# alvin-zyl/LDDL

Hardware: AMD Instinct MI355X
Metric: WordPiece tokens/sec (node) BERT seq128/512 at 1-8 GPUs; % HBM roofline (higher is better)
Workload: dtype u8

## Files before the change

lddl_amd/csrc/capi_tokenize.hip:

```cpp
#include "capi_ctx.h"

static int tok_debug_report(const TokParams& P, int64_t nt, hipStream_t st) {
  uint64_t h[24];
  HIP_TRY(hipMemcpyAsync(h, P.dbg, sizeof h, hipMemcpyDeviceToHost, st));
  HIP_TRY(hipStreamSynchronize(st));
  const char* nm[12] = {"loop", "setup", "classify", "except", "units", "urec", "prep", "probe", "records",
                        "tile_end", "entries", "tiles"};
  fprintf(stderr, "[lddl tok5 dbg] ntiles=%lld", (long long)nt);
  for (int k = 0; k < 12; ++k) fprintf(stderr, " %s=%llu", nm[k], (unsigned long long)h[k]);
  const char* wn[6] = {"wp_A", "wp_B", "wp_C", "wp_D", "wp_steps", "wp_lane_steps"};
  for (int k = 0; k < 6; ++k) fprintf(stderr, " %s=%llu", wn[k], (unsigned long long)h[12 + k]);
  fprintf(stderr, " prep_decode=%llu prep_dirty=%llu x_list=%llu x_load=%llu x_apply=%llu", (unsigned long long)h[18],
          (unsigned long long)h[19], (unsigned long long)h[20], (unsigned long long)h[21], (unsigned long long)h[22]);
  fprintf(stderr, "\n");
  return 0;
}

extern "C" int lddl_tokenize(lddl_ctx* c, const uint8_t* d_bytes, int64_t nbytes, const int64_t* d_sent_off,
                             int64_t n_sent, int32_t max_tok, uint16_t* d_out_ids, int64_t out_cap,
                             int32_t* d_out_ntok, int64_t* d_out_tok_off, void* stream) {
  if (!c) return set_err(LDDL_EINVAL, "null ctx");
  if (n_sent < 0 || max_tok < 1 || max_tok > 65534 || nbytes < 0 || out_cap < 0)
    return set_err(LDDL_EINVAL, "n_sent %lld nbytes %lld max_tok %d out_cap %lld", (long long)n_sent,
                   (long long)nbytes, max_tok, (long long)out_cap);
  if (!d_out_tok_off) return set_err(LDDL_EINVAL, "null device pointer");
  HIP_TRY(hipSetDevice(c->device));
  hipStream_t st = (hipStream_t)stream;
  if (n_sent == 0) {
    HIP_TRY(hipMemsetAsync(d_out_tok_off, 0, sizeof(int64_t), st));
    return 0;
  }
  if (!d_bytes || !d_sent_off || (!d_out_ids && out_cap > 0) || !d_out_ntok)
    return set_err(LDDL_EINVAL, "null device pointer");
  TokParams P{};
  P.bytes = d_bytes;
  P.sent_off = d_sent_off;
  P.n_sent = n_sent;
  P.max_tok = max_tok;
  P.out_ids = d_out_ids;
  P.out_ntok = d_out_ntok;
  P.out_tok_off = d_out_tok_off;
  P.out_cap = out_cap;
  c->spec_ids = nullptr;
  if (c->spec_flags) {
    int rc;
    if ((rc = ws_get(c, CW_SENT_SPEC, n_sent, &P.sent_spec))) return rc;
    c->spec_ids = d_out_ids;
    c->spec_ntok = d_out_ntok;
    c->spec_soff = d_sent_off;
    c->spec_nsent = n_sent;
  }
  P.top = c->d_top;
  P.pages = c->d_pages;
  P.bmp = c->d_bmp;
  P.xmap = c->d_xmap;
  P.multi = c->d_multi;
  P.slots = c->d_slots;
  P.slot_mask = c->slot_mask;
  P.bloom = c->d_bloom;
  P.pool = c->d_pool;
  P.voff = c->d_voff;
  P.maxb[0] = c->maxb[0];
  P.maxb[1] = c->maxb[1];
  for (int k = 0; k < 5; ++k) P.special[k] = c->special[k];
  P.unk = c->special[1];
  P.vt = c->d_vt;
  P.vt_mask = c->vt_mask;
  P.vbloom = c->d_vbloom;
  P.ovf = c->d_ovf;
  P.work_counter = c->d_counter;
  HIP_TRY(hipMemsetAsync(c->d_counter, 0, 64, st));
  const char* dbgenv = getenv("LDDL_TOK_DEBUG");

  if (dbgenv && dbgenv[0] == '1') {
    if (!c->d_tdbg) HIP_TRY(hipMalloc((void**)&c->d_tdbg, 32 * 8));
    HIP_TRY(hipMemsetAsync(c->d_tdbg, 0, 32 * 8, st));
    P.dbg = c->d_tdbg;
  }
  const int64_t nt = tile_count(nbytes);
  const char* eseg = getenv("LDDL_SPLIT_SEG");
  const char* ech = getenv("LDDL_SPLIT_CHUNKS");
  const int64_t seg_max = c->tok_algo == 0 ? nt : eseg && atoll(eseg) > 0 ? atoll(eseg) : SPLIT_SEG_TILES;
  const int64_t seg = nt < seg_max ? nt : seg_max;
  const bool split = c->tok_algo == 5;
  int64_t n_chunks = !split ? 1 : split_seg_slots(seg, c->n_cu) / SPLIT_CHUNK;
  if (ech && atoll(ech) > 0 && split) n_chunks = atoll(ech);
  const int64_t slots = n_chunks * SPLIT_CHUNK;
  int64_t* tile_sent;
  SplitParams S{};
  int rc;
  const int64_t fb_cap = fb_list_cap(seg, n_sent);
  if ((rc = ws_get(c, CW_TILE_SENT, nt + 1, &tile_sent)) || (rc = ws_get(c, CW_FB_LIST, (size_t)(2 * fb_cap), &S.fb_list)) ||
      (rc = ws_get(c, CW_FB_COUNT, 16, &S.fb_count)) ||
      (rc = ws_get(c, CW_ENT, (size_t)seg * 1024 + (size_t)max_tok + 4096, &S.ent)) ||
      (rc = ws_get(c, CW_SHARED_BSUM, (size_t)n_chunks + 16, &S.chunk_fill)) ||
      (rc = ws_get(c, CW_SCAN_BSUM, (size_t)scan_blocks(n_sent) + 1, &S.scan_bsum)))
// ... 27 lines not shown
```

lddl_amd/csrc/pack.hip:

```cpp
#include <algorithm>

#include "common.h"
#include "pack.h"
#include "pack_row.h"
#include "wave.h"

namespace lddl {

__global__ __launch_bounds__(1024) void scan_parts_kernel(const int64_t* a, const int64_t* b, int64_t n,
                                                          int64_t* sa, int64_t* sb, const int32_t* err,
                                                          int32_t* err_any) {
  __shared__ int64_t la[1024], lb[1024];
  __shared__ int32_t le;
  const int t = threadIdx.x;
  const int64_t per = (n + 1023) / 1024;
  const int64_t lo = min(n, t * per), hi = min(n, lo + per);
  int64_t x = 0, y = 0;
  int32_t e = 0;
  for (int64_t i = lo; i < hi; ++i) { x += a[i]; y += b[i]; e |= err[i]; }
  la[t] = x; lb[t] = y;
  if (t == 0) le = 0;
  __syncthreads();
  if (e) atomicOr(&le, e);
  for (int off = 1; off < 1024; off <<= 1) {
    int64_t u = t >= off ? la[t - off] : 0, w = t >= off ? lb[t - off] : 0;
    __syncthreads();
    la[t] += u; lb[t] += w;
    __syncthreads();
  }
  int64_t ra = la[t] - x, rb = lb[t] - y;
  for (int64_t i = lo; i < hi; ++i) { sa[i] = ra; sb[i] = rb; ra += a[i]; rb += b[i]; }
  if (t == 1023) { sa[n] = la[1023]; sb[n] = lb[1023]; *err_any = le; }
}

__global__ __launch_bounds__(256) void materialize_kernel(MatParams M) {
  __shared__ RowDesc st[4][64];
  __shared__ int64_t st_off[4][64];
  const PackView& V = M.V;
  const int lane = threadIdx.x & 63, wv = threadIdx.x >> 6;
  const int64_t total = V.pair_base[V.n_part];
  const int64_t nw = (int64_t)gridDim.x * 4;
  for (int64_t p = (int64_t)blockIdx.x * 4 + wv; p < V.n_part; p += nw) {
    const int64_t g0 = V.pair_base[p], np = V.pair_base[p + 1] - g0;
    for (int64_t c = 0; c < np; c += 64) {
      if (c + lane < np) {
        const int64_t g = g0 + c + lane;
        PairRec r;
        const RowRef w = pair_of_row(V, p, g, r);
        const int64_t off = row_tok_off(V, p, w);
        const RowDesc x = row_desc(V, r);
        st[wv][lane] = x;
        st_off[wv][lane] = off;
        store_row_meta(M, g, p, r.flags, x, total, [&] { return off; });
      }
      wave_sync();
      const int nr = (int)min((int64_t)64, np - c);
      const int hl = lane & 31;
      for (int r0 = 0; r0 < nr; r0 += 2) {
        const int rr = r0 + (lane >> 5);
        if (rr >= nr) continue;
        const RowDesc x = st[wv][rr];
        uint16_t* out = M.out_tokens + st_off[wv][rr];
        for (int t0 = 0; t0 < x.nt; t0 += 512) {
          uint16_t v[16];
#pragma unroll
          for (int k = 0; k < 16; ++k) {
            const int t = t0 + hl + 32 * k;
            uint16_t y = (uint16_t)M.sep_id;
            if (t == 0) y = (uint16_t)M.cls_id;
            else if (t <= x.l0) y = M.dense[x.src0 + (t - 1)];
            else if (t >= x.b1 && t < x.b1 + x.l1) y = M.dense[x.src1 + (t - x.b1)];
            v[k] = y;
          }
#pragma unroll
          for (int k = 0; k < 16; ++k) {
            const int t = t0 + hl + 32 * k;
            if (t < x.nt) out[t] = v[k];
          }
        }
      }
      wave_sync();
    }
  }
}

constexpr int MAT_U = 2;
constexpr int MAT_SLOW = 512;
// ... 176 lines not shown
}

hipError_t launch_chunk_parts(const int64_t* pair_base, const int64_t* doc_sent_off, const int64_t* part_doc_off,
                              int32_t dup, int64_t n_part, int32_t* chunk_part, int64_t* part_pb, hipStream_t s) {
  const int64_t nblk = std::max<int64_t>(1, std::min<int64_t>((n_part + 255) / 256, 1024));
  hipLaunchKernelGGL(chunk_parts_kernel, dim3((unsigned)nblk), dim3(256), 0, s, pair_base, doc_sent_off, part_doc_off,
                     dup, n_part, chunk_part, part_pb);
  return hipGetLastError();
}

constexpr int RS_U = 2;
__global__ __launch_bounds__(256) void rowspan_kernel(MatParams M, int64_t total) {
  const PackView& V = M.V;
  const int lane = threadIdx.x & 63, wv = threadIdx.x >> 6;
  const int64_t gbase = ((int64_t)blockIdx.x * 4 + wv) * 64 * RS_U;
  if (gbase >= total) return;
  int64_t g[RS_U], p[RS_U], at[RS_U];
  bool in[RS_U];
#pragma unroll
  for (int u = 0; u < RS_U; ++u) {
    g[u] = gbase + 64 * u + lane;
    in[u] = g[u] < total;
    p[u] = in[u] ? M.chunk_part[(gbase >> 6) + u] : 0;
  }
#pragma unroll
  for (int u = 0; u < RS_U; ++u) {
    if (in[u]) p[u] = part_walk(V, p[u], g[u]);
    at[u] = in[u] ? M.part_pb[p[u]] + (g[u] - V.pair_base[p[u]]) : 0;
  }
  SpanRec t[RS_U];
  int64_t off[RS_U];
#pragma unroll
  for (int u = 0; u < RS_U; ++u) t[u] = M.span[at[u]];
  if (M.out_tok_off) {
#pragma unroll
    for (int u = 0; u < RS_U; ++u) off[u] = V.tok_base[p[u]] + V.tok_local[at[u]];
  }
#pragma unroll
  for (int u = 0; u < RS_U; ++u) {
    if (!in[u]) continue;
    M.out_src0[g[u]] = t[u].src0;
    M.out_src1[g[u]] = t[u].src1;
    store_row_meta(M, g[u], p[u], t[u].flags, row_desc(t[u]), total, [&] { return off[u]; });
  }
}

hipError_t launch_row_spans(const MatParams& M, int64_t total_pairs, hipStream_t s) {
  const int64_t nblk = (total_pairs + 256 * RS_U - 1) / (256 * RS_U);
  hipLaunchKernelGGL(rowspan_kernel, dim3((unsigned)nblk), dim3(256), 0, s, M, total_pairs);
  return hipGetLastError();
}

constexpr int SCAN_ITEMS = 4096;

__host__ __device__ int64_t scan_blocks(int64_t n) { return (n + SCAN_ITEMS - 1) / SCAN_ITEMS; }

__device__ __forceinline__ int64_t block_excl_scan256(int64_t v, int64_t* red, int64_t* total) {
  const int lane = threadIdx.x & 63, w = threadIdx.x >> 6;
  int64_t x = v;
#pragma unroll
  for (int o = 1; o < 64; o <<= 1) {
    const int64_t y = __shfl_up(x, o);
    if (lane >= o) x += y;
  }
  if (lane == 63) red[w] = x;
  __syncthreads();
  int64_t pre = 0, tot = 0;
#pragma unroll
  for (int k = 0; k < 4; ++k) {
    if (k < w) pre += red[k];
    tot += red[k];
  }
  __syncthreads();
  *total = tot;
  return pre + x - v;
}

__device__ __forceinline__ void scan_range(const int64_t* d_lo, const int64_t* d_hi, int64_t n, int64_t& lo,
                                           int64_t& hi) {
  lo = d_lo ? *d_lo : 0;
  hi = d_lo ? *d_hi : n;
}

__global__ __launch_bounds__(256) void scan_reduce_kernel(const int32_t* ntok, const int64_t* d_lo, const int64_t* d_hi,
                                                          int64_t n, int64_t* bsum) {
  __shared__ int64_t red[4];
  int64_t lo, hi;
  scan_range(d_lo, d_hi, n, lo, hi);
  const int64_t b0 = lo + (int64_t)blockIdx.x * SCAN_ITEMS;
  if (b0 >= hi) return;
  int64_t sum = 0;
  for (int k = threadIdx.x; k < SCAN_ITEMS; k += 256)
    if (b0 + k < hi) sum += ntok[b0 + k];
  int64_t tot;
  block_excl_scan256(sum, red, &tot);
  if (threadIdx.x == 0) bsum[blockIdx.x] = tot;
}

__global__ __launch_bounds__(256) void scan_bsum_kernel(int64_t* bsum, const int64_t* d_lo, const int64_t* d_hi,
                                                        int64_t n, const int64_t* tokoff) {
  __shared__ int64_t red[4];
  int64_t lo, hi;
  scan_range(d_lo, d_hi, n, lo, hi);
  const int64_t nb = scan_blocks(hi - lo);
  int64_t carry = d_lo ? tokoff[lo] : 0;
  for (int64_t c = 0; c < nb; c += 256) {
    const int64_t i = c + threadIdx.x;
    const int64_t v = i < nb ? bsum[i] : 0;
    int64_t tot;
    const int64_t ex = block_excl_scan256(v, red, &tot);
    if (i < nb) bsum[i] = carry + ex;
    carry += tot;
  }
  if (threadIdx.x == 0) bsum[nb] = carry;
}

__global__ __launch_bounds__(256) void scan_write_kernel(const int32_t* ntok, const int64_t* d_lo, const int64_t* d_hi,
                                                         int64_t n, const int64_t* bsum, int64_t* tokoff) {
  __shared__ int64_t red[4];
  int64_t lo, hi;
  scan_range(d_lo, d_hi, n, lo, hi);
  if (lo + (int64_t)blockIdx.x * SCAN_ITEMS >= hi) return;
  const int64_t b0 = lo + (int64_t)blockIdx.x * SCAN_ITEMS + threadIdx.x * 16;
  int32_t v[16];
  int64_t sum = 0;
#pragma unroll
  for (int k = 0; k < 16; ++k) {
    v[k] = b0 + k < hi ? ntok[b0 + k] : 0;
    sum += v[k];
  }
  int64_t tot;
  int64_t run = bsum[blockIdx.x] + block_excl_scan256(sum, red, &tot);
  __shared__ int64_t ob[SCAN_ITEMS + SCAN_ITEMS / 16];
#pragma unroll
  for (int k = 0; k < 16; ++k) {
    ob[threadIdx.x * 17 + k] = run;
    run += v[k];
  }
  __syncthreads();
  const int64_t c0 = lo + (int64_t)blockIdx.x * SCAN_ITEMS;
#pragma unroll
  for (int k = 0; k < 16; ++k) {
    const int j = k * 256 + threadIdx.x;
    if (c0 + j < hi) tokoff[c0 + j] = ob[j + (j >> 4)];
  }
  if (lo + ((int64_t)blockIdx.x + 1) * SCAN_ITEMS >= hi && threadIdx.x == 0) tokoff[hi] = bsum[scan_blocks(hi - lo)];
}

static hipError_t scan_launch(const int32_t* ntok, const int64_t* d_lo, const int64_t* d_hi, int64_t n,
                              int64_t* tokoff, int64_t* blocksums, hipStream_t s) {
  const int64_t nb = scan_blocks(n);
  if (nb == 0) return d_lo ? hipSuccess : hipMemsetAsync(tokoff, 0, sizeof(int64_t), s);
  hipLaunchKernelGGL(scan_reduce_kernel, dim3((unsigned)nb), dim3(256), 0, s, ntok, d_lo, d_hi, n, blocksums);
  hipLaunchKernelGGL(scan_bsum_kernel, dim3(1), dim3(256), 0, s, blocksums, d_lo, d_hi, n, (const int64_t*)tokoff);
  hipLaunchKernelGGL(scan_write_kernel, dim3((unsigned)nb), dim3(256), 0, s, ntok, d_lo, d_hi, n,
                     (const int64_t*)blocksums, tokoff);
  return hipGetLastError();
}

hipError_t launch_scan_ntok(const int32_t* ntok, int64_t n, int64_t* tokoff, int64_t* blocksums, hipStream_t s) {
  return scan_launch(ntok, nullptr, nullptr, n, tokoff, blocksums, s);
}

hipError_t launch_scan_ntok_range(const int32_t* ntok, const int64_t* d_lo, const int64_t* d_hi, int64_t max_items,
                                  int64_t* tokoff, int64_t* blocksums, hipStream_t s) {
  return scan_launch(ntok, d_lo, d_hi, max_items, tokoff, blocksums, s);
}

hipError_t launch_scan_parts(const int64_t* a, const int64_t* b, int64_t n, int64_t* sa, int64_t* sb,
                             const int32_t* err, int32_t* err_any, hipStream_t s) {
  hipLaunchKernelGGL(scan_parts_kernel, dim3(1), dim3(1024), 0, s, a, b, n, sa, sb, err, err_any);
  return hipGetLastError();
}

__global__ __launch_bounds__(256) void sent_special_kernel(const uint16_t* ids, const int64_t* tok_off,
                                                           const int32_t* ntok, int64_t n_sent, uint32_t cls,
                                                           uint32_t sep, uint8_t* out) {
  for (int64_t s = (int64_t)blockIdx.x * blockDim.x + threadIdx.x; s < n_sent; s += (int64_t)gridDim.x * blockDim.x) {
    const uint16_t* t = ids + tok_off[s];
    const int n = ntok[s];
    uint32_t f = 0;
    for (int k = 0; k < n; ++k) {
      const uint32_t v = t[k];
      f |= (v == cls) | (v == sep);
    }
    out[s] = (uint8_t)f;
  }
}

__global__ __launch_bounds__(256) void masked_lm_kernel(MlmParams M) {
  const int sl = threadIdx.x & 15;
  const int64_t total = M.V.pair_base[M.V.n_part];
  const int64_t ng = (int64_t)gridDim.x * 16;
  for (int64_t g = (int64_t)blockIdx.x * 16 + (threadIdx.x >> 4); g < total; g += ng) {
    const int64_t p = M.row_part[g];
    const MaskRef m = mask_ref(M, p, row_ref(M.V, p, g));
    uint16_t* row = M.tokens + M.tok_off[g];
    if (sl == 0) store_mask_off(M, g, total, m);
    for (int k = sl; k < m.nm; k += 16) {
      const uint32_t e = M.marena[m.aoff + k];
      const uint32_t pos = e & 0xFFFFu, nid = e >> 16;
      const uint16_t label = row[pos];
      M.out_pos[m.ooff + k] = (uint16_t)pos;
      M.out_label[m.ooff + k] = label;
      if (nid != MLM_KEEP) row[pos] = (uint16_t)nid;
    }
  }
}

constexpr int MLM_SPAN_UNROLL = 8;

__global__ __launch_bounds__(256) void masked_lm_spans_kernel(MlmParams M) {
  struct RowLds {
    int64_t aoff[64], ooff[64], a[64], b[64];
    int32_t l0[64], pre[65];
  };
  __shared__ RowLds R[4];
  const int lane = threadIdx.x & 63, wv = threadIdx.x >> 6;
  RowLds& L = R[wv];
  const int64_t total = M.V.pair_base[M.V.n_part];
  const int64_t nw = (int64_t)gridDim.x * 4;
  for (int64_t g0 = ((int64_t)blockIdx.x * 4 + wv) * 64; g0 < total; g0 += nw * 64) {
    const int64_t g = g0 + lane;
    int nm = 0;
    if (g < total) {
      const int64_t p = M.row_part[g];
      const MaskRef m = mask_ref(M, p, row_ref(M.V, p, g));
      nm = m.nm;
      L.aoff[lane] = m.aoff;
      L.ooff[lane] = m.ooff;
      L.a[lane] = M.src0[g];
      L.b[lane] = M.src1[g];
      L.l0[lane] = M.len0[g];
      store_mask_off(M, g, total, m);
    }
    const int incl = wave_incl_add(nm);
    L.pre[lane] = incl - nm;
    if (lane == 63) L.pre[64] = incl;
    const int T = lane_get(incl, 63);
    wave_sync();
    int r = 0;
    constexpr int U = MLM_SPAN_UNROLL;
    for (int t0 = 0; t0 < T; t0 += 64 * U) {
      int rr[U], kk[U];
      uint32_t e[U];
#pragma unroll
      for (int u = 0; u < U; ++u) {
        const int t = t0 + 64 * u + lane;
        rr[u] = -1;
// ... 64 lines not shown
```

lddl_amd/csrc/tokenize.h:

```cpp
#pragma once
#include <hip/hip_runtime.h>
#include <stdint.h>

namespace lddl {

constexpr int WB_OVF = 384;
constexpr int TOK_WAVES = 4;
constexpr int BLOOM_WORDS = 8192;

struct TokParams {
  const uint8_t* bytes;
  const int64_t* sent_off;
  int64_t n_sent;
  int32_t max_tok;
  uint16_t* out_ids;
  int32_t* out_ntok;
  int64_t* out_tok_off;
  int64_t out_cap;
  uint8_t* sent_spec;
  const uint16_t* top;
  const uint32_t* pages;
  const uint4* multi;
  const uint32_t* bmp;
  const uint32_t* xmap;
  const uint4* slots;
  const uint32_t* bloom;
  uint32_t slot_mask;
  const uint8_t* pool;
  const uint32_t* voff;
  uint32_t maxb[2];
  uint32_t special[5];
  uint32_t unk;
  const uint4* vt;
  uint32_t vt_mask;
  const uint32_t* vbloom;
  uint8_t* ovf;
  uint32_t* work_counter;
  uint64_t* dbg;
};

int64_t tile_count(int64_t nbytes);
hipError_t launch_tile_bounds(const int64_t* sent_off, int64_t n_sent, int64_t n_tiles, int64_t* tile_sent,
                              hipStream_t s, int64_t seg = 0, int sup = 1);
hipError_t launch_tokenize_fallback(const TokParams& P, const int64_t* fb_list, const int32_t* fb_count,
                                    int64_t fb_cap, int grid, hipStream_t s);
const void* tokenize_fallback_kernel_ptr();
hipError_t launch_list_all_tiles(int64_t n_tiles, const int64_t* tile_sent, int64_t* fb_list, int32_t* fb_count,
                                 int64_t fb_cap, hipStream_t s);
inline int64_t fb_list_cap(int64_t seg_tiles, int64_t n_sent) {
  return 2 * seg_tiles + 64 + (n_sent + 30) / 31;
}

constexpr int64_t SPLIT_SEG_TILES = int64_t(1) << 23;
constexpr uint32_t SPLIT_CHUNK = 1024;
constexpr uint32_t SPLIT_EDEF = 0xF000u;
constexpr uint16_t SPLIT_NENT_FB = 0xFFFFu;
constexpr uint16_t SPLIT_EHOLE = 0xFFFFu;

struct SplitParams {
  int64_t seg_tiles;
  int64_t t0, t1;
  const int64_t* tile_sent;
  uint16_t* ent;
  uint4* rec;
  uint4* pcs;
  uint4* pch;
  uint32_t* chunk_fill;
  uint32_t* chunk_ctr;
  uint32_t n_chunks;
  uint2* smeta;
  uint16_t* snslot;
  uint8_t* cnt8;
  int64_t* scan_bsum;
  int64_t seg_sent_cap;
  int64_t* fb_list;
  int32_t* fb_count;
  int64_t fb_cap;
  uint32_t* n_fallback;
  unsigned long long* n_rec;
};
struct SplitTiming {
  hipEvent_t ev[3][2][64];
  int n[3];
};
hipError_t launch_tokenize_split(const TokParams& P, int64_t nbytes, int64_t* tile_sent, SplitParams S, int n_cu,
                                 int fb_grid, hipStream_t s, SplitTiming* tm = nullptr);
hipError_t launch_tokenize_serial_dense(const TokParams& P, int64_t nbytes, int64_t* tile_sent, SplitParams S,
                                        int n_cu, int fb_grid, hipStream_t s);
int64_t split_seg_slots(int64_t seg_tiles, int n_cu);

}
```

lddl_amd/csrc/tokenize_split.hip:

```cpp
#include <string.h>

#include "common.h"
#include "tokenize.h"
#include "wave.h"
#include "tokenize_serial.h"
#include "pack.h"


namespace lddl {
namespace tok5 {

constexpr int CAP = 2048;
constexpr int DCAP = 256;
constexpr int SCAN_OCC = 5;
#ifndef LDDL_SCAN_SUPER
#define LDDL_SCAN_SUPER 16
#endif
constexpr int SUPER = LDDL_SCAN_SUPER;
#ifndef LDDL_SCAN_FK
#define LDDL_SCAN_FK 2
#endif
constexpr int FK = LDDL_SCAN_FK;
#ifndef LDDL_SCAN_FKEY
#define LDDL_SCAN_FKEY 16
// ... 1219 lines not shown
        put_piece(0, (uint32_t)P.unk);
        np = 1;
        finish();
      } else {
        const int len = e - s;
        const int lc = min(len, 24);
        auto msk = [&](int k, uint32_t cc) {
          const int nbk = min(max(lc - 4 * k, 0), 4);
          return cc & (nbk >= 4 ? 0xFFFFFFFFu : ((1u << (8 * nbk)) - 1u));
        };
        const uint32_t m0c = msk(0, c0), m1c = msk(1, c1), m2c = msk(2, c2), m3c = msk(3, c3), m4c = msk(4, c4),
                       m5c = msk(5, c5);
        const uint32_t want = ((uint32_t)len << 16) | (cont << 24) | 0x80000000u;
        bool m0 = (((a1.z & 0xFFFF0000u) ^ want) | (a0.x ^ m0c) | (a0.y ^ m1c) | (a0.z ^ m2c) | (a0.w ^ m3c) |
                   (a1.x ^ m4c) | (a1.y ^ m5c)) == 0u;
        bool m1 = (((b1.z & 0xFFFF0000u) ^ want) | (b0.x ^ m0c) | (b0.y ^ m1c) | (b0.z ^ m2c) | (b0.w ^ m3c) |
                   (b1.x ^ m4c) | (b1.y ^ m5c)) == 0u;
        if (len > 24) {
          if (m0)
            for (int k = 24; k < len; ++k) m0 = m0 && kbyte(s + k) == P.pool[a1.w + k];
          if (m1)
            for (int k = 24; k < len; ++k) m1 = m1 && kbyte(s + k) == P.pool[b1.w + k];
        }
        if (m0 || m1) {
          put_piece(np, (m0 ? a1.z : b1.z) & 0xFFFFu);
          ++np;
          s = e;
          if (s >= we) {
            finish();
          } else {
            cont = 1;
            start_piece(mb1);
          }
        } else if (!(a1.z & 0x80000000u) || !(b1.z & 0x80000000u)) {
          bslot = -1;
          shrink();
        } else {
          bslot = (int)(((uint32_t)bslot + 1u) & vmask);
        }
      }
    }
    WP_STAMP(2)
    if (pr >= 0) {
      if (q0.x == 0u) {
        pr = -1;
      } else if ((q0.x & 0xFFu) > 24u && !qlong) {
        q2 = *recq(S, 2, (uint32_t)pr);
        q3 = *recq(S, 3, (uint32_t)pr);
        qlong = true;
      } else if (r < 0) {
        const int len = (int)(q0.x & 0xFFu);
        kb[0] = q0.z; kb[64] = q0.w;
        kb[128] = q1.x; kb[192] = q1.y; kb[256] = q1.z; kb[320] = q1.w;
        kb[384] = q2.x; kb[448] = q2.y; kb[512] = q2.z; kb[576] = q2.w;
        kb[640] = q3.x; kb[704] = q3.y; kb[768] = q3.z; kb[832] = q3.w;
        kb[896] = 0u;
        kb[960] = 0u;
        r = pr;
        pr = -1;
        ++nrec;
        s = 0;
        we = len;
        np = 0;
        cont = 0;
        start_piece(mb0);
      }
    }
    WP_STAMP(3)
    if (wdbg) {
      wacc[4] += 1;
      wacc[5] += __popcll(__ballot(r >= 0));
    }
    if (__ballot(r >= 0 || pr >= 0) == 0 && u >= nun) break;
  }
  if (wdbg && lane == 0)
    for (int k = 0; k < 6; ++k) atomicAdd((unsigned long long*)&P.dbg[12 + k], (unsigned long long)wacc[k]);
#undef WP_STAMP
  if (S.n_rec) {
    const uint32_t tot = lane_get(wave_incl_add(nrec), 63);
    if (lane == 0 && tot) atomicAdd(S.n_rec, (unsigned long long)tot);
  }
}

constexpr int CNT_U = 4;
__global__ __launch_bounds__(256) void count_kernel(TokParams P, SplitParams S) {
  const int64_t sA = S.tile_sent[S.t0], sB = S.tile_sent[S.t1];
  const int64_t stride = (int64_t)gridDim.x * 256 * CNT_U;
  for (int64_t s0 = sA + (int64_t)blockIdx.x * 256 * CNT_U + threadIdx.x; s0 < sB; s0 += stride) {
    uint2 m[CNT_U];
    int32_t t[CNT_U];
    uint32_t n[CNT_U];
#pragma unroll
    for (int u = 0; u < CNT_U; ++u) {
      const int64_t s = s0 + 256 * u;
      const bool in = s < sB;
      m[u] = in ? S.smeta[s] : make_uint2(SPLIT_NENT_FB, 0u);
      t[u] = in ? P.out_ntok[s] : 0;
      n[u] = in ? S.snslot[s] : 0u;
    }
#pragma unroll
    for (int u = 0; u < CNT_U; ++u) {
      if ((m[u].x & 0xFFFFu) != SPLIT_NENT_FB) {
        const uint32_t q = m[u].y + (m[u].x >> 16);
        for (uint32_t k = 0; k < n[u]; ++k) t[u] += S.cnt8[q + k];
        t[u] = min(t[u], P.max_tok);
      }
    }
#pragma unroll
    for (int u = 0; u < CNT_U; ++u)
      if (s0 + 256 * u < sB) P.out_ntok[s0 + 256 * u] = t[u];
  }
}

struct ExpSent {
  int64_t eb;
  int64_t dst;
  uint32_t qb;
  uint32_t lim;
  uint32_t e0;
  uint32_t pad;
};
struct ExpLds {
  ExpSent sn[64];
  uint32_t hf[64];
};

template <bool ALL_DIRECT>
__global__ __launch_bounds__(256) void expand_kernel(TokParams P, SplitParams S) {
  __shared__ ExpLds X[4];
  const int lane = threadIdx.x & 63;
  const int wv = __builtin_amdgcn_readfirstlane(threadIdx.x >> 6);
  ExpLds& E = X[wv];
  const int64_t sA = uni64(S.tile_sent[S.t0]), sB = uni64(S.tile_sent[S.t1]);
  const int64_t base = P.sent_off[0], ebase = S.t0 << 10;
  const int64_t nwaves = (int64_t)gridDim.x * 4;
  typedef uint32_t u32x3 __attribute__((ext_vector_type(3)));
  const uint4* const pcs = S.pcs;
  const uint4* const pch = S.pch;
  uint32_t tag = 0;
  E.hf[lane] = 0u;
  for (int64_t g0 = sA + ((int64_t)blockIdx.x * 4 + wv) * 64; g0 < sB; g0 += nwaves * 64) {
    const int64_t s = g0 + lane;
    uint32_t ne = 0;
    int64_t eoff = 0, d = 0;
    uint32_t qb = 0, lim = 0;
    if (s < sB) {
      const uint2 m = S.smeta[s];
      const int32_t nt = P.out_ntok[s];
      ne = m.x & 0xFFFFu;
      if (ne == SPLIT_NENT_FB) ne = (uint32_t)nt;
      d = P.out_tok_off[s];
      eoff = P.sent_off[s] - base - ebase;
      qb = (m.x & 0xFFFFu) == SPLIT_NENT_FB ? 0u : m.y;
      lim = (uint32_t)max((int64_t)0, min((int64_t)nt, P.out_cap - d));
    }
    const uint32_t x = wave_incl_add(ne);
    const uint32_t e0 = x - ne;
    const uint32_t T = lane_get(x, 63);
    ExpSent es;
    es.eb = eoff - (int64_t)e0;
    es.dst = d;
    es.qb = qb;
    es.lim = lim;
    es.e0 = e0;
    es.pad = 0;
    const uint64_t nzm = __ballot(ne != 0);
    if (ne != 0) E.sn[bits_below(nzm)] = es;
    uint32_t hcar = 0;
    auto owner = [&](uint32_t st) -> uint32_t {
      ++tag;
      if (ne != 0 && e0 - st < 64u) E.hf[e0 - st] = tag;
      wsync();
      const bool head = E.hf[lane] == tag;
      const uint64_t hm = __ballot(head);
      const uint32_t o = hcar + (uint32_t)bits_below(hm) + (head ? 0u : (uint32_t)-1);
      hcar += (uint32_t)__popcll(hm);
      return o;
    };
#ifndef LDDL_EXP_K
#define LDDL_EXP_K 5
#endif
    constexpr int EXP_K = LDDL_EXP_K;
    uint32_t carry = 0;
    for (uint32_t st0 = 0; st0 < T; st0 += 64 * EXP_K) {
      uint32_t xj[EXP_K], xv[EXP_K];
      bool xin[EXP_K];
#pragma unroll
      for (int k = 0; k < EXP_K; ++k) {
        const uint32_t st = st0 + 64 * k;
        xj[k] = 0;
        xv[k] = 0;
        xin[k] = false;
        if (st < T) {
          const uint32_t g = st + (uint32_t)lane;
          xj[k] = min(owner(st), 63u);
          xin[k] = g < T;
          const ExpSent sj = E.sn[xj[k]];
          xv[k] = S.ent[xin[k] ? sj.eb + g : 0];
        }
      }
      u32x3 xr[EXP_K];
#pragma unroll
      for (int k = 0; k < EXP_K; ++k) {
        const bool r = !ALL_DIRECT && xin[k] && xv[k] >= SPLIT_EDEF && xv[k] != SPLIT_EHOLE;
        xr[k] = u32x3{0u, 0u, 0u};
        if (st0 + 64 * k < T)
          xr[k] = *reinterpret_cast<const u32x3*>(pch + (r ? (size_t)(E.sn[xj[k]].qb + (xv[k] & 0xFFFu)) : 0));
      }
#pragma unroll
      for (int k = 0; k < EXP_K; ++k) {
        const uint32_t st = st0 + 64 * k;
        if (st >= T) break;
        const uint32_t cj = xj[k], cv = xin[k] ? xv[k] : 0u;
        const bool cin = xin[k], rec = !ALL_DIRECT && cin && cv >= SPLIT_EDEF && cv != SPLIT_EHOLE;
        const u32x3 rq = rec ? xr[k] : u32x3{cin && (ALL_DIRECT || cv != SPLIT_EHOLE) ? 1u : 0u, 0u, 0u};
        const ExpSent sj = E.sn[cj];
        const size_t ri = (size_t)(sj.qb + (cv & 0xFFFu)) * 4;
        const uint32_t cnt = rq.x;
        const uint32_t xex = wave_incl_add(cnt) - cnt;
        const int hl = (int)(sj.e0 - st);
        const uint32_t hb = (uint32_t)__shfl((int)xex, hl & 63);
        const uint32_t p = xex - (hl >= 0 ? hb : 0u - carry);
        const int room = (int)sj.lim - (int)p;
        const uint32_t nw = room > 0 ? min(cnt, (uint32_t)room) : 0u;
        if (nw) {
          uint16_t* o = P.out_ids + sj.dst + p;
          o[0] = (uint16_t)(ALL_DIRECT || cv < SPLIT_EDEF ? cv : rq.y & 0xFFFFu);
          if (nw > 1) o[1] = (uint16_t)(rq.y >> 16);
          if (nw > 2) o[2] = (uint16_t)(rq.z & 0xFFFFu);
          if (nw > 3) o[3] = (uint16_t)(rq.z >> 16);
          if (nw > 4) {
            const uint16_t* pc = reinterpret_cast<const uint16_t*>(pcs + ri);
            for (uint32_t q = 4; q < nw; ++q) o[q] = pc[piece_at((int)q)];
          }
        }
        const uint32_t ll = min(T, st + 64) - 1 - st;
        carry = lane_get(p + cnt, (int)ll);
      }
    }
    wsync();
  }
}

template <int WAVES, bool DBG, int OCC>
static hipError_t launch_scan(const TokParams& P, const SplitParams& S, int n_cu, hipStream_t s) {
  static int per_cu = 0;
  if (per_cu == 0 &&
      (hipOccupancyMaxActiveBlocksPerMultiprocessor(&per_cu, scan_kernel<WAVES, DBG, OCC>, 64 * WAVES, 0) !=
           hipSuccess ||
       per_cu < 1))
    per_cu = 1;
  int64_t grid = (int64_t)n_cu * per_cu;
  const int64_t ng = (S.t1 - S.t0 + SUPER - 1) / SUPER;
  const int64_t need = (ng + WAVES - 1) / WAVES;
  if (grid > need) grid = need;
  if (grid < 1) grid = 1;
  hipLaunchKernelGGL((scan_kernel<WAVES, DBG, OCC>), dim3((unsigned)grid), dim3(64 * WAVES), 0, s, P, S);
  return hipGetLastError();
}

template <int WAVES>
static hipError_t launch_wp(const TokParams& P, const SplitParams& S, int n_cu, hipStream_t s) {
  static int per_cu = 0;
  if (per_cu == 0 &&
      (hipOccupancyMaxActiveBlocksPerMultiprocessor(&per_cu, wp_kernel<WAVES>, 64 * WAVES, 0) != hipSuccess ||
       per_cu < 1))
    per_cu = 1;
  const int64_t grid = (int64_t)n_cu * per_cu;
  hipLaunchKernelGGL(wp_kernel<WAVES>, dim3((unsigned)grid), dim3(64 * WAVES), 0, s, P, S);
  return hipGetLastError();
}

}

constexpr int SCAN_WAVES = 4, WP_WAVES = 12;
hipError_t finish_segment(TokParams P, const SplitParams& S, int n_cu, int fb_grid, hipStream_t s, bool all_direct = false);

int64_t split_seg_slots(int64_t seg_tiles, int n_cu) {
  int per_cu = 0;
  if (hipOccupancyMaxActiveBlocksPerMultiprocessor(&per_cu, tok5::scan_kernel<SCAN_WAVES, false, tok5::SCAN_OCC>, 64 * SCAN_WAVES,
                                                   0) != hipSuccess || per_cu < 1)
    per_cu = 8;
  const int64_t waves = (int64_t)n_cu * per_cu * SCAN_WAVES;
  const int64_t chunks = (seg_tiles * 1024 / 14 + SPLIT_CHUNK - 1) / SPLIT_CHUNK + std::min(waves, seg_tiles) + 16;
  return chunks * SPLIT_CHUNK;
}

__global__ void smeta_fallback_kernel(uint2* smeta, int64_t n_sent) {
  for (int64_t s = (int64_t)blockIdx.x * blockDim.x + threadIdx.x; s < n_sent; s += (int64_t)gridDim.x * blockDim.x)
    smeta[s] = make_uint2(SPLIT_NENT_FB, 0xFFFFFFFFu);
}

hipError_t launch_tokenize_serial_dense(const TokParams& P, int64_t nbytes, int64_t* tile_sent, SplitParams S,
                                        int n_cu, int fb_grid, hipStream_t s) {
  const int64_t n_tiles = tile_count(nbytes);
  hipError_t e = launch_tile_bounds(P.sent_off, P.n_sent, n_tiles, tile_sent, s);
  if (e != hipSuccess || (e = hipMemsetAsync(P.out_tok_off, 0, sizeof(int64_t), s)) != hipSuccess) return e;
  S.tile_sent = tile_sent;
  S.t0 = 0;
  S.t1 = n_tiles;
  if ((e = launch_list_all_tiles(n_tiles, tile_sent, S.fb_list, S.fb_count, S.fb_cap, s)) != hipSuccess) return e;
  hipLaunchKernelGGL(smeta_fallback_kernel, dim3(1024), dim3(256), 0, s, S.smeta, P.n_sent);
  if ((e = hipGetLastError()) != hipSuccess) return e;
  return finish_segment(P, S, n_cu, fb_grid, s, true);
}

hipError_t launch_tokenize_split(const TokParams& P, int64_t nbytes, int64_t* tile_sent, SplitParams S, int n_cu,
                                 int fb_grid, hipStream_t s, SplitTiming* tm) {
  if (tm) tm->n[0] = tm->n[1] = tm->n[2] = 0;
  auto mark = [&](int k, int side) -> hipError_t {
    if (!tm || tm->n[k] >= 64) return hipSuccess;
    const hipError_t e = hipEventRecord(tm->ev[k][side][tm->n[k]], s);
    if (side == 1) ++tm->n[k];
    return e;
  };
  const int64_t n_tiles = tile_count(nbytes);
  const int64_t seg = S.seg_tiles > 0 ? S.seg_tiles : SPLIT_SEG_TILES;
  hipError_t e = launch_tile_bounds(P.sent_off, P.n_sent, n_tiles, tile_sent, s, seg, tok5::SUPER);
  if (e != hipSuccess) return e;
  if ((e = hipMemsetAsync(P.out_tok_off, 0, sizeof(int64_t), s)) != hipSuccess) return e;
  S.tile_sent = tile_sent;
  for (int64_t t0 = 0; t0 < n_tiles; t0 += seg) {
    S.t0 = t0;
    S.t1 = std::min(n_tiles, t0 + seg);
    if ((e = hipMemsetAsync(S.chunk_ctr, 0, 12, s)) != hipSuccess) return e;
    if ((e = hipMemsetAsync(S.fb_count, 0, 4, s)) != hipSuccess) return e;
    if ((e = mark(0, 0)) != hipSuccess) return e;
    if (P.dbg) e = tok5::launch_scan<SCAN_WAVES, true, tok5::SCAN_OCC>(P, S, n_cu, s);
    else e = tok5::launch_scan<SCAN_WAVES, false, tok5::SCAN_OCC>(P, S, n_cu, s);
    if (e != hipSuccess || (e = mark(0, 1)) != hipSuccess || (e = mark(1, 0)) != hipSuccess) return e;
    if ((e = tok5::launch_wp<WP_WAVES>(P, S, n_cu, s)) != hipSuccess) return e;
    if ((e = mark(1, 1)) != hipSuccess || (e = mark(2, 0)) != hipSuccess) return e;
    if ((e = finish_segment(P, S, n_cu, fb_grid, s)) != hipSuccess || (e = mark(2, 1)) != hipSuccess) return e;
  }
  return hipSuccess;
}

hipError_t finish_segment(TokParams P, const SplitParams& S, int n_cu, int fb_grid, hipStream_t s, bool all_direct) {
  TokParams F = P;
  F.out_ids = S.ent - (S.t0 << 10);
  hipError_t e = launch_tokenize_fallback(F, S.fb_list, S.fb_count, S.fb_cap, fb_grid, s);
  if (e != hipSuccess) return e;
#ifndef LDDL_CNT_BLOCKS
#define LDDL_CNT_BLOCKS 256
#endif
  const int64_t cnt_grid = std::max<int64_t>(
      1, std::min<int64_t>((int64_t)n_cu * LDDL_CNT_BLOCKS, (S.seg_sent_cap + 256 * tok5::CNT_U - 1) / (256 * tok5::CNT_U)));
  hipLaunchKernelGGL(tok5::count_kernel, dim3((unsigned)cnt_grid), dim3(256), 0, s, P, S);
  if ((e = hipGetLastError()) != hipSuccess) return e;
  if ((e = launch_scan_ntok_range(P.out_ntok, S.tile_sent + S.t0, S.tile_sent + S.t1, S.seg_sent_cap, P.out_tok_off,
                                  S.scan_bsum, s)) != hipSuccess)
    return e;
  static const int exp_blocks = [] {
    const char* v = getenv("LDDL_EXP_BLOCKS");
    const int b = v ? atoi(v) : 0;
    return b > 0 && b <= 4096 ? b : 192;
  }();
  const int64_t exp_grid = std::max<int64_t>(1, std::min<int64_t>((int64_t)n_cu * exp_blocks, (S.seg_sent_cap + 255) / 256));
  if (all_direct) hipLaunchKernelGGL(tok5::expand_kernel<true>, dim3((unsigned)exp_grid), dim3(256), 0, s, P, S);
  else hipLaunchKernelGGL(tok5::expand_kernel<false>, dim3((unsigned)exp_grid), dim3(256), 0, s, P, S);
  return hipGetLastError();
}

}
```

Measured before the change: 47.13 billion.

## Fuse token count into scan reduce and software-pipeline expand entry loads

Removes the separate count_kernel and folds the per-sentence piece-count accumulation and max_tok clamp into the scan reduce pass, saving one launch and one read/write pass over ntok. The expand kernel now prefetches the next batch's entry values while the current batch's record loads are in flight, packs owner indices into one register, and requests a fixed 8 waves per EU. It also adds optional s_memtime phase stamps for debugging. The risks are higher register pressure from the pipelining and a reduce grid that is now sized by scan blocks rather than the old count grid.

```diff
diff --git a/lddl_amd/csrc/capi_tokenize.hip b/lddl_amd/csrc/capi_tokenize.hip
--- a/lddl_amd/csrc/capi_tokenize.hip
+++ b/lddl_amd/csrc/capi_tokenize.hip
@@ -1,7 +1,7 @@
 #include "capi_ctx.h"
 
 static int tok_debug_report(const TokParams& P, int64_t nt, hipStream_t st) {
-  uint64_t h[24];
+  uint64_t h[32];
   HIP_TRY(hipMemcpyAsync(h, P.dbg, sizeof h, hipMemcpyDeviceToHost, st));
   HIP_TRY(hipStreamSynchronize(st));
   const char* nm[12] = {"loop", "setup", "classify", "except", "units", "urec", "prep", "probe", "records",
@@ -12,6 +12,10 @@
   for (int k = 0; k < 6; ++k) fprintf(stderr, " %s=%llu", wn[k], (unsigned long long)h[12 + k]);
   fprintf(stderr, " prep_decode=%llu prep_dirty=%llu x_list=%llu x_load=%llu x_apply=%llu", (unsigned long long)h[18],
           (unsigned long long)h[19], (unsigned long long)h[20], (unsigned long long)h[21], (unsigned long long)h[22]);
+  if (h[24] | h[28]) {
+    const char* en[7] = {"header", "owner_issue", "entry_wait", "rec_issue", "rec_wait", "tokens", "stores"};
+    for (int k = 0; k < 7; ++k) fprintf(stderr, " exp_%s=%llu", en[k], (unsigned long long)h[24 + k]);
+  }
   fprintf(stderr, "\n");
   return 0;
 }
diff --git a/lddl_amd/csrc/pack.hip b/lddl_amd/csrc/pack.hip
--- a/lddl_amd/csrc/pack.hip
+++ b/lddl_amd/csrc/pack.hip
@@ -3,6 +3,7 @@
 #include "common.h"
 #include "pack.h"
 #include "pack_row.h"
+#include "tokenize.h"
 #include "wave.h"
 
 namespace lddl {
@@ -345,16 +346,59 @@
   hi = d_lo ? *d_hi : n;
 }
 
-__global__ __launch_bounds__(256) void scan_reduce_kernel(const int32_t* ntok, const int64_t* d_lo, const int64_t* d_hi,
-                                                          int64_t n, int64_t* bsum) {
+constexpr int SCAN_CNT_U = 4;
+template <bool COUNT>
+__global__ __launch_bounds__(256) void scan_reduce_kernel(int32_t* ntok, const int64_t* d_lo, const int64_t* d_hi,
+                                                          int64_t n, int64_t* bsum, ScanCount C) {
   __shared__ int64_t red[4];
   int64_t lo, hi;
   scan_range(d_lo, d_hi, n, lo, hi);
   const int64_t b0 = lo + (int64_t)blockIdx.x * SCAN_ITEMS;
   if (b0 >= hi) return;
   int64_t sum = 0;
-  for (int k = threadIdx.x; k < SCAN_ITEMS; k += 256)
-    if (b0 + k < hi) sum += ntok[b0 + k];
+  if constexpr (!COUNT) {
+    for (int k = threadIdx.x; k < SCAN_ITEMS; k += 256)
+      if (b0 + k < hi) sum += ntok[b0 + k];
+  } else {
+    for (int k = threadIdx.x; k < SCAN_ITEMS; k += 256 * SCAN_CNT_U) {
+      uint2 m[SCAN_CNT_U];
+      int32_t t[SCAN_CNT_U];
+      uint32_t ns[SCAN_CNT_U];
+#pragma unroll
+      for (int u = 0; u < SCAN_CNT_U; ++u) {
+        const int64_t s = b0 + k + 256 * u;
+        const bool in = s < hi;
+        m[u] = in ? C.smeta[s] : make_uint2(SPLIT_NENT_FB, 0u);
+        t[u] = in ? ntok[s] : 0;
+        ns[u] = in ? C.snslot[s] : 0u;
+      }
+      uint32_t q[SCAN_CNT_U], nmax = 0;
+#pragma unroll
+      for (int u = 0; u < SCAN_CNT_U; ++u) {
+        if ((m[u].x & 0xFFFFu) == SPLIT_NENT_FB) ns[u] = 0;
+        q[u] = m[u].y + (m[u].x >> 16);
+        nmax = max(nmax, ns[u]);
+      }
+      for (uint32_t j = 0; j < nmax; j += 2) {
+        uint32_t c[SCAN_CNT_U][2];
+#pragma unroll
+        for (int u = 0; u < SCAN_CNT_U; ++u) {
+          c[u][0] = j < ns[u] ? C.cnt8[q[u] + j] : 0u;
+          c[u][1] = j + 1 < ns[u] ? C.cnt8[q[u] + j + 1] : 0u;
+        }
+#pragma unroll
+        for (int u = 0; u < SCAN_CNT_U; ++u) t[u] += (int32_t)(c[u][0] + c[u][1]);
+      }
+#pragma unroll
+      for (int u = 0; u < SCAN_CNT_U; ++u)
+        if ((m[u].x & 0xFFFFu) != SPLIT_NENT_FB) t[u] = min(t[u], C.max_tok);
+#pragma unroll
+      for (int u = 0; u < SCAN_CNT_U; ++u) {
+        if (b0 + k + 256 * u < hi) ntok[b0 + k + 256 * u] = t[u];
+        sum += t[u];
+      }
+    }
+  }
   int64_t tot;
   block_excl_scan256(sum, red, &tot);
   if (threadIdx.x == 0) bsum[blockIdx.x] = tot;
@@ -410,24 +454,30 @@
   if (lo + ((int64_t)blockIdx.x + 1) * SCAN_ITEMS >= hi && threadIdx.x == 0) tokoff[hi] = bsum[scan_blocks(hi - lo)];
 }
 
-static hipError_t scan_launch(const int32_t* ntok, const int64_t* d_lo, const int64_t* d_hi, int64_t n,
-                              int64_t* tokoff, int64_t* blocksums, hipStream_t s) {
+template <bool COUNT>
+static hipError_t scan_launch(int32_t* ntok, const int64_t* d_lo, const int64_t* d_hi, int64_t n, int64_t* tokoff,
+                              int64_t* blocksums, hipStream_t s, const ScanCount& C = ScanCount{}) {
   const int64_t nb = scan_blocks(n);
   if (nb == 0) return d_lo ? hipSuccess : hipMemsetAsync(tokoff, 0, sizeof(int64_t), s);
-  hipLaunchKernelGGL(scan_reduce_kernel, dim3((unsigned)nb), dim3(256), 0, s, ntok, d_lo, d_hi, n, blocksums);
+  hipLaunchKernelGGL(scan_reduce_kernel<COUNT>, dim3((unsigned)nb), dim3(256), 0, s, ntok, d_lo, d_hi, n, blocksums, C);
   hipLaunchKernelGGL(scan_bsum_kernel, dim3(1), dim3(256), 0, s, blocksums, d_lo, d_hi, n, (const int64_t*)tokoff);
-  hipLaunchKernelGGL(scan_write_kernel, dim3((unsigned)nb), dim3(256), 0, s, ntok, d_lo, d_hi, n,
+  hipLaunchKernelGGL(scan_write_kernel, dim3((unsigned)nb), dim3(256), 0, s, (const int32_t*)ntok, d_lo, d_hi, n,
                      (const int64_t*)blocksums, tokoff);
   return hipGetLastError();
 }
 
 hipError_t launch_scan_ntok(const int32_t* ntok, int64_t n, int64_t* tokoff, int64_t* blocksums, hipStream_t s) {
-  return scan_launch(ntok, nullptr, nullptr, n, tokoff, blocksums, s);
+  return scan_launch<false>(const_cast<int32_t*>(ntok), nullptr, nullptr, n, tokoff, blocksums, s);
 }
 
 hipError_t launch_scan_ntok_range(const int32_t* ntok, const int64_t* d_lo, const int64_t* d_hi, int64_t max_items,
                                   int64_t* tokoff, int64_t* blocksums, hipStream_t s) {
-  return scan_launch(ntok, d_lo, d_hi, max_items, tokoff, blocksums, s);
+  return scan_launch<false>(const_cast<int32_t*>(ntok), d_lo, d_hi, max_items, tokoff, blocksums, s);
+}
+
+hipError_t launch_scan_count_range(int32_t* ntok, const ScanCount& C, const int64_t* d_lo, const int64_t* d_hi,
+                                   int64_t max_items, int64_t* tokoff, int64_t* blocksums, hipStream_t s) {
+  return scan_launch<true>(ntok, d_lo, d_hi, max_items, tokoff, blocksums, s, C);
 }
 
 hipError_t launch_scan_parts(const int64_t* a, const int64_t* b, int64_t n, int64_t* sa, int64_t* sb,
diff --git a/lddl_amd/csrc/tokenize.h b/lddl_amd/csrc/tokenize.h
--- a/lddl_amd/csrc/tokenize.h
+++ b/lddl_amd/csrc/tokenize.h
@@ -79,6 +79,14 @@
   uint32_t* n_fallback;
   unsigned long long* n_rec;
 };
+struct ScanCount {
+  const uint2* smeta;
+  const uint16_t* snslot;
+  const uint8_t* cnt8;
+  int32_t max_tok;
+};
+hipError_t launch_scan_count_range(int32_t* ntok, const ScanCount& C, const int64_t* d_lo, const int64_t* d_hi,
+                                   int64_t max_items, int64_t* tokoff, int64_t* blocksums, hipStream_t s);
 struct SplitTiming {
   hipEvent_t ev[3][2][64];
   int n[3];
diff --git a/lddl_amd/csrc/tokenize_split.hip b/lddl_amd/csrc/tokenize_split.hip
--- a/lddl_amd/csrc/tokenize_split.hip
+++ b/lddl_amd/csrc/tokenize_split.hip
@@ -1325,36 +1325,6 @@
   }
 }
 
-constexpr int CNT_U = 4;
-__global__ __launch_bounds__(256) void count_kernel(TokParams P, SplitParams S) {
-  const int64_t sA = S.tile_sent[S.t0], sB = S.tile_sent[S.t1];
-  const int64_t stride = (int64_t)gridDim.x * 256 * CNT_U;
-  for (int64_t s0 = sA + (int64_t)blockIdx.x * 256 * CNT_U + threadIdx.x; s0 < sB; s0 += stride) {
-    uint2 m[CNT_U];
-    int32_t t[CNT_U];
-    uint32_t n[CNT_U];
-#pragma unroll
-    for (int u = 0; u < CNT_U; ++u) {
-      const int64_t s = s0 + 256 * u;
-      const bool in = s < sB;
-      m[u] = in ? S.smeta[s] : make_uint2(SPLIT_NENT_FB, 0u);
-      t[u] = in ? P.out_ntok[s] : 0;
-      n[u] = in ? S.snslot[s] : 0u;
-    }
-#pragma unroll
-    for (int u = 0; u < CNT_U; ++u) {
-      if ((m[u].x & 0xFFFFu) != SPLIT_NENT_FB) {
-        const uint32_t q = m[u].y + (m[u].x >> 16);
-        for (uint32_t k = 0; k < n[u]; ++k) t[u] += S.cnt8[q + k];
-        t[u] = min(t[u], P.max_tok);
-      }
-    }
-#pragma unroll
-    for (int u = 0; u < CNT_U; ++u)
-      if (s0 + 256 * u < sB) P.out_ntok[s0 + 256 * u] = t[u];
-  }
-}
-
 struct ExpSent {
   int64_t eb;
   int64_t dst;
@@ -1368,9 +1338,28 @@
   uint32_t hf[64];
 };
 
+#ifdef LDDL_EXP_STAMP
+#define EXP_STAMP(k)                                    \
+  {                                                     \
+    const uint64_t t_ = __builtin_amdgcn_s_memtime();   \
+    ph[k] += t_ - tprev;                                \
+    tprev = t_;                                         \
+  }
+#define EXP_WAIT_STAMP(k)                 \
+  {                                       \
+    __builtin_amdgcn_s_waitcnt(0x0F70);   \
+    EXP_STAMP(k)                          \
+  }
+#else
+#define EXP_STAMP(k)
+#define EXP_WAIT_STAMP(k)
+#endif
 template <bool ALL_DIRECT>
-__global__ __launch_bounds__(256) void expand_kernel(TokParams P, SplitParams S) {
+__attribute__((amdgpu_waves_per_eu(8, 8))) __global__ __launch_bounds__(256) void expand_kernel(TokParams P, SplitParams S) {
   __shared__ ExpLds X[4];
+#ifdef LDDL_EXP_STAMP
+  uint64_t ph[7] = {0, 0, 0, 0, 0, 0, 0}, tprev = __builtin_amdgcn_s_memtime();
+#endif
   const int lane = threadIdx.x & 63;
   const int wv = __builtin_amdgcn_readfirstlane(threadIdx.x >> 6);
   ExpLds& E = X[wv];
@@ -1409,6 +1398,7 @@
     es.pad = 0;
     const uint64_t nzm = __ballot(ne != 0);
     if (ne != 0) E.sn[bits_below(nzm)] = es;
+    EXP_WAIT_STAMP(0)
     uint32_t hcar = 0;
     auto owner = [&](uint32_t st) -> uint32_t {
       ++tag;
@@ -1423,39 +1413,72 @@
 #ifndef LDDL_EXP_K
 #define LDDL_EXP_K 5
 #endif
+#ifndef LDDL_EXP_PIPE
+#define LDDL_EXP_PIPE 1
+#endif
     constexpr int EXP_K = LDDL_EXP_K;
+    static_assert(EXP_K >= 1 && EXP_K <= 5, "a batch's sentence ranks are 6 bits each in one register");
+    constexpr bool PIPE = LDDL_EXP_PIPE != 0;
+    auto load_entries = [&](uint32_t b0, uint32_t (&v)[EXP_K], uint32_t& jp) {
+      jp = 0;
+#pragma unroll
+      for (int k = 0; k < EXP_K; ++k) {
+        const uint32_t st = b0 + 64 * k;
+        const uint32_t g = st + (uint32_t)lane;
+        int64_t at = 0;
+        if (st < T) {
+          const uint32_t j = min(owner(st), 63u);
+          jp |= j << (6 * k);
+          if (g < T) at = E.sn[j].eb + g;
+        }
+        v[k] = S.ent[at];
+      }
+    };
     uint32_t carry = 0;
+    uint32_t xv[EXP_K], xjp = 0;
+    if (PIPE && T != 0) load_entries(0, xv, xjp);
+    EXP_STAMP(1)
     for (uint32_t st0 = 0; st0 < T; st0 += 64 * EXP_K) {
-      uint32_t xj[EXP_K], xv[EXP_K];
-      bool xin[EXP_K];
+      if (!PIPE) {
+        load_entries(st0, xv, xjp);
+        EXP_STAMP(1)
+      }
+      {
+        uint32_t any = 0;
+#pragma unroll
+        for (int k = 0; k < EXP_K; ++k) any |= xv[k];
+        asm volatile("" ::"v"(any));
+      }
+      EXP_STAMP(2)
+      u32x3 xr[EXP_K];
 #pragma unroll
       for (int k = 0; k < EXP_K; ++k) {
-        const uint32_t st = st0 + 64 * k;
-        xj[k] = 0;
-        xv[k] = 0;
-        xin[k] = false;
-        if (st < T) {
-          const uint32_t g = st + (uint32_t)lane;
-          xj[k] = min(owner(st), 63u);
-          xin[k] = g < T;
-          const ExpSent sj = E.sn[xj[k]];
-          xv[k] = S.ent[xin[k] ? sj.eb + g : 0];
-        }
-      }
-      u32x3 xr[EXP_K];
-#pragma unroll
-      for (int k = 0; k < EXP_K; ++k) {
-        const bool r = !ALL_DIRECT && xin[k] && xv[k] >= SPLIT_EDEF && xv[k] != SPLIT_EHOLE;
+        const bool xin = st0 + 64 * k + (uint32_t)lane < T;
+        const bool r = !ALL_DIRECT && xin && xv[k] >= SPLIT_EDEF && xv[k] != SPLIT_EHOLE;
         xr[k] = u32x3{0u, 0u, 0u};
-        if (st0 + 64 * k < T)
-          xr[k] = *reinterpret_cast<const u32x3*>(pch + (r ? (size_t)(E.sn[xj[k]].qb + (xv[k] & 0xFFFu)) : 0));
-      }
+        if (!ALL_DIRECT && st0 + 64 * k < T)
+          xr[k] = *reinterpret_cast<const u32x3*>(pch + (r ? (size_t)(E.sn[(xjp >> (6 * k)) & 63u].qb + (xv[k] & 0xFFFu)) : 0));
+      }
+      EXP_STAMP(3)
+      uint32_t nv[EXP_K], njp = 0;
+      if (PIPE) {
+        load_entries(st0 + 64 * EXP_K, nv, njp);
+        EXP_STAMP(1)
+      }
+      if (!ALL_DIRECT) {
+        uint32_t any = 0;
+#pragma unroll
+        for (int k = 0; k < EXP_K; ++k) any |= xr[k].x;
+        asm volatile("" ::"v"(any));
+      }
+      EXP_STAMP(4)
 #pragma unroll
       for (int k = 0; k < EXP_K; ++k) {
         const uint32_t st = st0 + 64 * k;
         if (st >= T) break;
-        const uint32_t cj = xj[k], cv = xin[k] ? xv[k] : 0u;
-        const bool cin = xin[k], rec = !ALL_DIRECT && cin && cv >= SPLIT_EDEF && cv != SPLIT_EHOLE;
+        const bool cin = st + (uint32_t)lane < T;
+        const uint32_t cj = (xjp >> (6 * k)) & 63u, cv = cin ? xv[k] : 0u;
+        const bool rec = !ALL_DIRECT && cin && cv >= SPLIT_EDEF && cv != SPLIT_EHOLE;
         const u32x3 rq = rec ? xr[k] : u32x3{cin && (ALL_DIRECT || cv != SPLIT_EHOLE) ? 1u : 0u, 0u, 0u};
         const ExpSent sj = E.sn[cj];
         const size_t ri = (size_t)(sj.qb + (cv & 0xFFFu)) * 4;
@@ -1466,6 +1489,7 @@
         const uint32_t p = xex - (hl >= 0 ? hb : 0u - carry);
         const int room = (int)sj.lim - (int)p;
         const uint32_t nw = room > 0 ? min(cnt, (uint32_t)room) : 0u;
+        EXP_STAMP(5)
         if (nw) {
           uint16_t* o = P.out_ids + sj.dst + p;
           o[0] = (uint16_t)(ALL_DIRECT || cv < SPLIT_EDEF ? cv : rq.y & 0xFFFFu);
@@ -1477,13 +1501,26 @@
             for (uint32_t q = 4; q < nw; ++q) o[q] = pc[piece_at((int)q)];
           }
         }
+        EXP_STAMP(6)
         const uint32_t ll = min(T, st + 64) - 1 - st;
         carry = lane_get(p + cnt, (int)ll);
       }
+      EXP_STAMP(5)
+      if (PIPE) {
+#pragma unroll
+        for (int k = 0; k < EXP_K; ++k) xv[k] = nv[k];
+        xjp = njp;
+      }
     }
     wsync();
   }
-}
+#ifdef LDDL_EXP_STAMP
+  if (P.dbg && lane == 0)
+    for (int k = 0; k < 7; ++k) atomicAdd((unsigned long long*)&P.dbg[24 + k], (unsigned long long)ph[k]);
+#endif
+}
+#undef EXP_STAMP
+#undef EXP_WAIT_STAMP
 
 template <int WAVES, bool DBG, int OCC>
 static hipError_t launch_scan(const TokParams& P, const SplitParams& S, int n_cu, hipStream_t s) {
@@ -1584,15 +1621,9 @@
   F.out_ids = S.ent - (S.t0 << 10);
   hipError_t e = launch_tokenize_fallback(F, S.fb_list, S.fb_count, S.fb_cap, fb_grid, s);
   if (e != hipSuccess) return e;
-#ifndef LDDL_CNT_BLOCKS
-#define LDDL_CNT_BLOCKS 256
-#endif
-  const int64_t cnt_grid = std::max<int64_t>(
-      1, std::min<int64_t>((int64_t)n_cu * LDDL_CNT_BLOCKS, (S.seg_sent_cap + 256 * tok5::CNT_U - 1) / (256 * tok5::CNT_U)));
-  hipLaunchKernelGGL(tok5::count_kernel, dim3((unsigned)cnt_grid), dim3(256), 0, s, P, S);
-  if ((e = hipGetLastError()) != hipSuccess) return e;
-  if ((e = launch_scan_ntok_range(P.out_ntok, S.tile_sent + S.t0, S.tile_sent + S.t1, S.seg_sent_cap, P.out_tok_off,
-                                  S.scan_bsum, s)) != hipSuccess)
+  const ScanCount C{S.smeta, S.snslot, S.cnt8, P.max_tok};
+  if ((e = launch_scan_count_range(P.out_ntok, C, S.tile_sent + S.t0, S.tile_sent + S.t1, S.seg_sent_cap, P.out_tok_off,
+                                   S.scan_bsum, s)) != hipSuccess)
     return e;
   static const int exp_blocks = [] {
     const char* v = getenv("LDDL_EXP_BLOCKS");
```

Result: no change. 47.96 billion, median of 6 (+1.8%).
